# regicide211212/multi-style-transfer-gan

Measured on AMD Instinct MI355X. Metric: train-step images/sec (fwd+bwd+loss), 256x256 batch32, higher is better.
Workload: dtype f32; 1 GPU; config 3: reference CycleGAN train_step (2x EnhancedGenerator + 2x EnhancedDiscriminator, channels=16, num_transformer_blocks=0), 32 image pairs/GPU at 256x256, fwd+bwd+loss+Adam; per_gpu_batch=32, size=256, channels=16, parallelism=dp1, collective=none, losses_finite=True

## Files before the change

multi-style-transfer-gan_amd/mstg_hip/csrc/common.h:

```cpp
#pragma once
#include <hip/hip_runtime.h>
#include <stdint.h>
#include <stdio.h>
#include <string.h>

#include "mstg_hip.h"

typedef float f32x4 __attribute__((ext_vector_type(4)));
typedef float f32x2 __attribute__((ext_vector_type(2)));

namespace mstg {

extern thread_local char g_last_error[256];
inline int fail_launch(hipError_t e, const char* what) {
    snprintf(g_last_error, sizeof(g_last_error), "%s: %s", what, hipGetErrorString(e));
    return MSTG_E_LAUNCH;
}
inline int fail_arg(int code, const char* what) {
    snprintf(g_last_error, sizeof(g_last_error), "%s", what);
    return code;
}
#define MSTG_CHECK_LAUNCH(what)                                   \
    do {                                                          \
        hipError_t e__ = hipGetLastError();                       \
        if (e__ != hipSuccess) return mstg::fail_launch(e__, what); \
    } while (0)

extern bool g_prof_on;
void prof_begin(const void* host_fn, hipStream_t st);
void prof_end(hipStream_t st);
#define MSTG_LAUNCH(kern, grid, block, lds, st, ...)                               \
    do {                                                                           \
        const bool prof__ = mstg::g_prof_on;                                       \
        if (prof__) mstg::prof_begin((const void*)(kern), (hipStream_t)(st));      \
        hipLaunchKernelGGL(kern, grid, block, lds, st, __VA_ARGS__);               \
        if (prof__) mstg::prof_end((hipStream_t)(st));                             \
    } while (0)

extern thread_local bool t_ws_packed;
#define MSTG_PACK_LAUNCH(...)                      \
    do {                                           \
        if (!mstg::t_ws_packed) MSTG_LAUNCH(__VA_ARGS__); \
    } while (0)

enum EnvKnob {
    ENV_ATTN_BLK4, ENV_ATTN_BLK64, ENV_WGRAD_1X1, ENV_WGRAD_TS_MAXCH, ENV_WGRAD_PLAIN, ENV_WGRAD_OLD, ENV_NO_DPACK, ENV_IGEMM,
    ENV_STREAM, ENV_PF, ENV_WGLOB, ENV_HEAVY_PER_CU, ENV_DBG, ENV_DBG_LDS_KB, ENV_MS_WGRAD_PACKED, ENV_MS_FWD4, ENV_NO_PACK_CACHE,
    ENV_P32, ENV_P32_TH, ENV_P32_WLDS, ENV_P32_DBG, ENV_P32_OCC, ENV_ATTN_REG, ENV_NFW_ADAPT, ENV_BSUMS_ALL, ENV_ATTN_BIG32, ENV_NORM_WGS,
    ENV_CONV_IMG, ENV_COUNT
};
const char* env_get(EnvKnob k);

int cu_count();
struct OccCache {
    const void* kern = nullptr;
    size_t lds = 0;
    int occ = 1;
};
int persistent_occupancy(OccCache& c, const void* kern, size_t lds);

constexpr int WAVE = 64;

__device__ __forceinline__ f32x4 mfma16(float a, float b, f32x4 c) {
    return __builtin_amdgcn_mfma_f32_16x16x4f32(a, b, c, 0, 0, 0);
}

__device__ __forceinline__ float wave_sum(float v) {
#pragma unroll
    for (int o = 32; o > 0; o >>= 1) v += __shfl_xor(v, o, 64);
    return v;
}

__device__ __forceinline__ float apply_act(float v, int act) {
    switch (act) {
        case MSTG_ACT_RELU: return v > 0.f ? v : 0.f;
        case MSTG_ACT_LEAKY02: return v > 0.f ? v : 0.2f * v;
        case MSTG_ACT_TANH: return tanhf(v);
        case MSTG_ACT_GELU: return 0.5f * v * (1.f + erff(v * 0.70710678118654752f));
        default: return v;
    }
}
__device__ __forceinline__ float act_grad(float v, int act) {
    switch (act) {
        case MSTG_ACT_RELU: return v > 0.f ? 1.f : 0.f;
        case MSTG_ACT_LEAKY02: return v > 0.f ? 1.f : 0.2f;
        case MSTG_ACT_TANH: return 1.f - v * v;
        case MSTG_ACT_GELU: return 0.5f * (1.f + erff(v * 0.70710678118654752f)) + v * 0.3989422804014327f * expf(-0.5f * v * v);
        default: return 1.f;
    }
}

__device__ __forceinline__ int xcd_swizzle(int bid, int nblk) {
    const int q = nblk >> 3, r = nblk & 7, xcd = bid & 7, k = bid >> 3;
    return (xcd < r ? xcd * (q + 1) : r * (q + 1) + (xcd - r) * q) + k;
}


__host__ __device__ __forceinline__ unsigned magic_u32(unsigned d) { return 0xFFFFFFFFu / d + 1u; }

template <int NB>
__device__ __forceinline__ void stage_window_batch(const float* __restrict__ img, float* __restrict__ lds, int total, int e0, int cols,
                                                   int nq, unsigned m_cols, unsigned m_nq, int y0, int x0, int H, int W, int ctot,
                                                   int nq_valid, int ckp, int tid, int rowpad) {
    f32x4 v[NB];
    int dst[NB];
    bool ok[NB];
#pragma unroll
    for (int k = 0; k < NB; ++k) {
        const int e = e0 + 256 * k + tid;
        const int p = nq == 1 ? e : (int)__umulhi((unsigned)e, m_nq);
        const int q = e - p * nq;
        const int r = (int)__umulhi((unsigned)p, m_cols), c = p - r * cols;
        const int iy = y0 + r, ix = x0 + c;
        ok[k] = e < total && (unsigned)iy < (unsigned)H && (unsigned)ix < (unsigned)W && q < nq_valid;
        const unsigned off = ok[k] ? (unsigned)(iy * W + ix) * (unsigned)ctot + 4u * q : 0u;
        v[k] = *reinterpret_cast<const f32x4*>(img + off);
        dst[k] = e < total ? p * ckp + 4 * q + r * rowpad : -1;
    }
#pragma unroll
    for (int k = 0; k < NB; ++k)
        if (dst[k] >= 0) *reinterpret_cast<f32x4*>(&lds[dst[k]]) = ok[k] ? v[k] : f32x4{0.f, 0.f, 0.f, 0.f};
}

__device__ __forceinline__ void stage_window(const float* __restrict__ img, float* __restrict__ lds, int rows, int cols, int nq,
                                             unsigned m_cols, unsigned m_nq, int y0, int x0, int H, int W, int ctot, int nq_valid,
                                             int ckp, int tid, int rowpad = 0) {
    const int total = rows * cols * nq;
    int e0 = 0;
    for (; e0 + 1024 < total; e0 += 2048)
        stage_window_batch<8>(img, lds, total, e0, cols, nq, m_cols, m_nq, y0, x0, H, W, ctot, nq_valid, ckp, tid, rowpad);
    for (; e0 < total; e0 += 1024)
        stage_window_batch<4>(img, lds, total, e0, cols, nq, m_cols, m_nq, y0, x0, H, W, ctot, nq_valid, ckp, tid, rowpad);
// ... 38 lines not shown
```

multi-style-transfer-gan_amd/mstg_hip/csrc/msblock.hip:

```cpp
#include "common.h"
#include <stdlib.h>

namespace mstg {

constexpr int MS_TH = 8, MS_PH = MS_TH + 8, MS_PW = 16 + 8, MS_CKP = 20;

template <int CH>
__global__ __launch_bounds__(256) void wgrad_ms_kernel(const float* __restrict__ x, const float* __restrict__ dy,
                                                       float* __restrict__ partial, int N, int H, int W, int tiles_x, int tiles_y,
                                                       int ntiles) {
    constexpr int NFH = CH / 16, C4 = CH / 4, U = NFH + 24, UW = (U + 3) / 4, BNP = CH + 4, NG = CH / 16;
    constexpr int PSTRIDE = NG * U * 256 + CH;
    extern __shared__ __attribute__((aligned(16))) float smem[];
    float* patch = smem;
    float* ht = smem + MS_PH * MS_PW * MS_CKP;

    const int tid = threadIdx.x, lane = tid & 63, wave = tid >> 6, i = lane & 15, g = lane >> 4;
    const int gchunk = blockIdx.y, g0 = 16 * gchunk;

    f32x4 acc[UW];
    int toff[UW], hfo[UW];
#pragma unroll
    for (int k = 0; k < UW; ++k) {
        const int u = min(wave + 4 * k, U - 1);
        int dyp = 0, dxp = 0, frag = u;
        if (u >= NFH) {
            const int r = (u - NFH) >> 3, i8 = (u - NFH) & 7, t9 = i8 < 4 ? i8 : i8 + 1, d = 1 << r;
            dyp = (t9 / 3 - 1) * d;
            dxp = (t9 % 3 - 1) * d;
            frag = ((r + 1) * C4) / 16;
        }
        toff[k] = ((4 + dyp) * MS_PW + 4 + dxp) * MS_CKP;
        hfo[k] = 16 * frag;
        acc[k] = f32x4{0.f, 0.f, 0.f, 0.f};
    }
    const int nu = (U - wave + 3) / 4;

    const bool do_bias = gchunk == 0;
    float bsum = 0.f;
    const unsigned m_pw = magic_u32(MS_PW), m_nq = magic_u32(CH / 4);
    const size_t plane = (size_t)H * W;
    for (int tile = blockIdx.x; tile < ntiles; tile += gridDim.x) {
        const int tx0 = tile % tiles_x, ty0 = (tile / tiles_x) % tiles_y, n = tile / (tiles_x * tiles_y);
        __syncthreads();
        stage_window(x + (size_t)n * plane * CH + g0, patch, MS_PH, MS_PW, 4, m_pw, 0x40000000u, ty0 * MS_TH - 4, tx0 * 16 - 4, H, W, CH, 4,
                     MS_CKP, tid);
        stage_window(dy + (size_t)n * plane * CH, ht, MS_TH, 16, CH / 4, 0x10000000u, m_nq, ty0 * MS_TH, tx0 * 16, H, W, CH, CH / 4, BNP, tid);
        __syncthreads();
        if (do_bias && tid < CH) {
#pragma unroll 8
            for (int p = 0; p < MS_TH * 16; ++p) bsum += ht[p * BNP + tid];
        }
#pragma unroll 1
        for (int r = 0; r < MS_TH; ++r) {
#pragma unroll 2
            for (int xs = 0; xs < 4; ++xs) {
                const int c = 4 * xs + g;
                const int abase = (r * MS_PW + c) * MS_CKP + i;
                const int hbase = (r * 16 + c) * BNP + i;
                float af[UW], bf[UW];
#pragma unroll
                for (int k = 0; k < UW; ++k) { af[k] = patch[abase + toff[k]]; bf[k] = ht[hbase + hfo[k]]; }
#pragma unroll
                for (int k = 0; k < UW; ++k) acc[k] = mfma16(af[k], bf[k], acc[k]);
            }
        }
    }
    float* out = partial + (size_t)blockIdx.x * PSTRIDE;
    if (do_bias && tid < CH) out[NG * U * 256 + tid] = bsum;
#pragma unroll
    for (int k = 0; k < UW; ++k) {
        if (k >= nu) continue;
        const int u = wave + 4 * k;
        float* o = out + ((size_t)gchunk * U + u) * 256;
#pragma unroll
        for (int e = 0; e < 4; ++e) o[(4 * g + e) * 16 + i] = acc[k][e];
    }
}

template <int CH>
struct MsUnits {
    static constexpr int NFW = CH / 16, C4 = CH / 4, U = NFW + 24;
    __host__ __device__ static constexpr int ring(int u) { return (u - NFW) >> 3; }
    __host__ __device__ static constexpr int t9(int u) { return ((u - NFW) & 7) < 4 ? ((u - NFW) & 7) : ((u - NFW) & 7) + 1; }
    __host__ __device__ static constexpr int oy(int u) { return u < NFW ? 0 : (t9(u) / 3 - 1) * (1 << ring(u)); }
    __host__ __device__ static constexpr int ox(int u) { return u < NFW ? 0 : (t9(u) % 3 - 1) * (1 << ring(u)); }
    __host__ __device__ static constexpr int frag(int u) { return u < NFW ? u : ((ring(u) + 1) * C4) / 16; }
};

struct MsParamPtrs {
    const float* w[4];
// ... 146 lines not shown
        for (int wf = 0; wf < NFW; ++wf) a[wf] = *reinterpret_cast<const f32x4*>(wpc + ((wf * K::NQ + Q) * 64 + lane) * 4);
#pragma unroll
        for (int e = 0; e < 4; ++e) {
            constexpr int s0 = 4 * Q;
            const int s = s0 + e;
            if (s < K::NS) {
                const int off = (K::oy(s) * MS_PW + K::ox(s)) * MS_CKP + 4 * K::grp(s);
                float b[2];
#pragma unroll
                for (int pf = 0; pf < 2; ++pf) b[pf] = patch[pbase + pf * MS_PW * MS_CKP + off];
#pragma unroll
                for (int wf = 0; wf < NFW; ++wf)
#pragma unroll
                    for (int pf = 0; pf < 2; ++pf) acc[wf][pf] = mfma16(a[wf][e], b[pf], acc[wf][pf]);
            }
        }
        MsDgQuadLoop<CH, C, QB + 1, QE>::run(acc, wpc, patch, pbase, lane);
    }
};
template <int CH, int C, int QE>
struct MsDgQuadLoop<CH, C, QE, QE> {
    template <typename ACC>
    static __device__ __forceinline__ void run(ACC&, const float*, const float*, int, int) {}
};

template <int CH, int C, typename ACC>
__device__ __forceinline__ void ms_dgrad_chunk(ACC& acc, const float* __restrict__ dy_img, const float* __restrict__ wp, float* patch,
                                               int ty0, int tx0, int H, int W, unsigned m_pw, int pbase, int tid, int lane) {
    typedef MsDgChunk<CH, C> K;
    constexpr int NFW = CH / 16;
    if (C) __syncthreads();
    stage_window(dy_img + 16 * C, patch, MS_PH, MS_PW, 4, m_pw, 0x40000000u, ty0 * MS_TH - 4, tx0 * 16 - 4, H, W, CH, 4, MS_CKP, tid);
    __syncthreads();
    MsDgQuadLoop<CH, C, 0, K::NQ>::run(acc, wp + (size_t)ms_dg_quads_before<CH>(C) * NFW * 256, patch, pbase, lane);
}

template <int CH>
__global__ __launch_bounds__(256) void ms_dgrad_kernel(const float* __restrict__ dy, const float* __restrict__ wp,
                                                       const float* __restrict__ dres, float* __restrict__ dx, int N, int H, int W,
                                                       int tiles_x, int tiles_y) {
    constexpr int NFW = CH / 16, PF = 2;
    extern __shared__ __attribute__((aligned(16))) float smem[];
    float* patch = smem;
    const int tid = threadIdx.x, lane = tid & 63, wave = tid >> 6, i = lane & 15, g = lane >> 4;
    const int tile = xcd_swizzle(blockIdx.x, gridDim.x);
    const int tx0 = tile % tiles_x, ty0 = (tile / tiles_x) % tiles_y, n = tile / (tiles_x * tiles_y);
    const size_t plane = (size_t)H * W;
    const unsigned m_pw = magic_u32(MS_PW);
    f32x4 acc[NFW][PF];
#pragma unroll
    for (int wf = 0; wf < NFW; ++wf)
#pragma unroll
        for (int pf = 0; pf < PF; ++pf) acc[wf][pf] = f32x4{0.f, 0.f, 0.f, 0.f};
    const int pbase = ((PF * wave + 4) * MS_PW + i + 4) * MS_CKP + g;
    const float* dy_img = dy + (size_t)n * plane * CH;
    ms_dgrad_chunk<CH, 0>(acc, dy_img, wp, patch, ty0, tx0, H, W, m_pw, pbase, tid, lane);
    if (CH >= 32) ms_dgrad_chunk<CH, (CH >= 32 ? 1 : 0)>(acc, dy_img, wp, patch, ty0, tx0, H, W, m_pw, pbase, tid, lane);
    if (CH >= 64) {
        ms_dgrad_chunk<CH, (CH >= 64 ? 2 : 0)>(acc, dy_img, wp, patch, ty0, tx0, H, W, m_pw, pbase, tid, lane);
        ms_dgrad_chunk<CH, (CH >= 64 ? 3 : 0)>(acc, dy_img, wp, patch, ty0, tx0, H, W, m_pw, pbase, tid, lane);
    }
#pragma unroll
    for (int pf = 0; pf < PF; ++pf) {
        const int gy = ty0 * MS_TH + PF * wave + pf, gx = tx0 * 16 + i;
        if (gy < H && gx < W) {
            const size_t o = (((size_t)n * H + gy) * W + gx) * CH + 4 * g;
#pragma unroll
            for (int wf = 0; wf < NFW; ++wf) {
                f32x4 v = acc[wf][pf];
                if (dres) v += *reinterpret_cast<const f32x4*>(dres + o + 16 * wf);
                *reinterpret_cast<f32x4*>(dx + o + 16 * wf) = v;
            }
        }
    }
}

template <int CH>
struct MsPk {
    static constexpr int NFH = CH / 16, C4 = CH / 4, TPU = 16 / C4, UPB = 8 / TPU, U = NFH + 3 * UPB, UW = (U + 3) / 4;
    static constexpr int NG = CH / 16, PSTRIDE = NG * U * 256 + CH, LDY = CH + 4;
};

template <int CH>
__global__ __launch_bounds__(256) void wgrad_msp_kernel(const float* __restrict__ x, const float* __restrict__ dy,
                                                        float* __restrict__ partial, int N, int H, int W, int tiles_x, int tiles_y,
                                                        int ntiles) {
    typedef MsPk<CH> G;
    constexpr int UW = G::UW, U = G::U, LDY = G::LDY, MG = G::NG, LDX = CH + 4;
    extern __shared__ __attribute__((aligned(16))) float smem[];
    float* xs = smem;
    float* dyp = smem + MS_TH * 16 * LDX;

    const int tid = threadIdx.x, lane = tid & 63, wave = tid >> 6, i = lane & 15, g = lane >> 4;

    f32x4 acc[UW][MG];
    int boff[UW];
#pragma unroll
    for (int k = 0; k < UW; ++k) {
        const int u = min(wave + 4 * k, U - 1);
        int off;
        if (u < G::NFH) {
            off = 16 * u + i;
        } else {
            const int j = 1 + (u - G::NFH) / G::UPB, m = (u - G::NFH) % G::UPB;
            const int sidx = i / G::C4, co = i % G::C4, i8 = m * G::TPU + sidx, t9 = i8 < 4 ? i8 : i8 + 1, d = 1 << (j - 1);
            const int oy = (t9 / 3 - 1) * d, ox = (t9 % 3 - 1) * d;
            off = (-oy * MS_PW - ox) * LDY + j * G::C4 + co;
        }
        boff[k] = off;
#pragma unroll
        for (int mf = 0; mf < MG; ++mf) acc[k][mf] = f32x4{0.f, 0.f, 0.f, 0.f};
    }
    const int nu = (U - wave + 3) / 4;

    float bsum = 0.f;
    const unsigned m_pw = magic_u32(MS_PW), m_nq = magic_u32(CH / 4);
    const size_t plane = (size_t)H * W;
    for (int tile = blockIdx.x; tile < ntiles; tile += gridDim.x) {
        const int tx0 = tile % tiles_x, ty0 = (tile / tiles_x) % tiles_y, n = tile / (tiles_x * tiles_y);
        __syncthreads();
        stage_window(x + (size_t)n * plane * CH, xs, MS_TH, 16, CH / 4, 0x10000000u, m_nq, ty0 * MS_TH, tx0 * 16, H, W, CH, CH / 4, LDX, tid);
        stage_window(dy + (size_t)n * plane * CH, dyp, MS_PH, MS_PW, CH / 4, m_pw, m_nq, ty0 * MS_TH - 4, tx0 * 16 - 4, H, W, CH, CH / 4, LDY,
                     tid);
        __syncthreads();
        if (tid < CH) {
            for (int r = 0; r < MS_TH; ++r)
#pragma unroll 8
                for (int c = 0; c < 16; ++c) bsum += dyp[((r + 4) * MS_PW + c + 4) * LDY + tid];
        }
#pragma unroll 1
        for (int r = 0; r < MS_TH; ++r) {
#pragma unroll 2
            for (int xs4 = 0; xs4 < 4; ++xs4) {
                const int c = 4 * xs4 + g;
                float af[MG], bf[UW];
#pragma unroll
                for (int mf = 0; mf < MG; ++mf) af[mf] = xs[(r * 16 + c) * LDX + 16 * mf + i];
                const int bbase = ((r + 4) * MS_PW + c + 4) * LDY;
#pragma unroll
                for (int k = 0; k < UW; ++k) bf[k] = dyp[bbase + boff[k]];
#pragma unroll
                for (int k = 0; k < UW; ++k)
#pragma unroll
                    for (int mf = 0; mf < MG; ++mf) acc[k][mf] = mfma16(af[mf], bf[k], acc[k][mf]);
            }
        }
    }
    float* out = partial + (size_t)blockIdx.x * G::PSTRIDE;
    if (tid < CH) out[G::NG * U * 256 + tid] = bsum;
#pragma unroll
    for (int k = 0; k < UW; ++k) {
        if (k >= nu) continue;
        const int u = wave + 4 * k;
#pragma unroll
        for (int mf = 0; mf < MG; ++mf) {
            float* o = out + ((size_t)mf * U + u) * 256;
#pragma unroll
            for (int e = 0; e < 4; ++e) o[(4 * g + e) * 16 + i] = acc[k][mf][e];
        }
    }
}

constexpr int M4_TH = 16, M4_PH = M4_TH + 8;

template <int CH, int JB, int T9, int Q>
struct Ms4Step {
    static constexpr int C4 = CH / 4, RS = C4 / 4;
    static __device__ __forceinline__ void run(f32x4 (&acc)[4][RS], const float* __restrict__ wl, const float* __restrict__ patch, int pbase,
                                               int wbase) {
        constexpr int d = JB == 0 ? 0 : (1 << (JB - 1));
        constexpr int oy = JB == 0 ? 0 : (T9 / 3 - 1) * d, ox = JB == 0 ? 0 : (T9 % 3 - 1) * d;
        constexpr int t = JB == 0 ? 0 : 1 + 9 * (JB - 1) + T9;
        const f32x4 b = *reinterpret_cast<const f32x4*>(&patch[pbase + (oy * MS_PW + ox) * MS_CKP + 4 * Q]);
#pragma unroll
        for (int rs = 0; rs < RS; ++rs) {
            const f32x4 a = *reinterpret_cast<const f32x4*>(&wl[wbase + (t * C4 + 4 * rs) * CH + 4 * Q]);
#pragma unroll
            for (int e = 0; e < 4; ++e) acc[JB][rs] = __builtin_amdgcn_mfma_f32_4x4x1f32(a[e], b[e], acc[JB][rs], 0, 0, 0);
        }
    }
};

template <int CH, int JB>
struct Ms4Branch {
    static constexpr int RS = CH / 16;
    static __device__ __forceinline__ void run(f32x4 (&acc)[4][RS], const float* wl, const float* patch, int pbase, int wbase) {
#define M4_TAP(T9)                                                  \
    Ms4Step<CH, JB, T9, 0>::run(acc, wl, patch, pbase, wbase);      \
    Ms4Step<CH, JB, T9, 1>::run(acc, wl, patch, pbase, wbase);      \
    Ms4Step<CH, JB, T9, 2>::run(acc, wl, patch, pbase, wbase);      \
    Ms4Step<CH, JB, T9, 3>::run(acc, wl, patch, pbase, wbase);
        if (JB == 0) {
            M4_TAP(0)
        } else {
            M4_TAP(0) M4_TAP(1) M4_TAP(2) M4_TAP(3) M4_TAP(4) M4_TAP(5) M4_TAP(6) M4_TAP(7) M4_TAP(8)
        }
#undef M4_TAP
    }
};

template <int CH>
__global__ __launch_bounds__(256) void ms_fwd4_kernel(const float* __restrict__ x, MsParamPtrs prm, float* __restrict__ y, int N, int H,
                                                      int W, int tiles_x, int tiles_y) {
    constexpr int C4 = CH / 4, RS = C4 / 4, NCHK = CH / 16;
    extern __shared__ __attribute__((aligned(16))) float smem[];
    float* patch = smem;
    float* wl = smem + M4_PH * MS_PW * MS_CKP;
    const int tid = threadIdx.x, lane = tid & 63, wave = tid >> 6;
    const int tile = xcd_swizzle(blockIdx.x, gridDim.x);
    const int tx0 = tile % tiles_x, ty0 = (tile / tiles_x) % tiles_y, n = tile / (tiles_x * tiles_y);
    const size_t plane = (size_t)H * W;
    for (int e = tid; e < 28 * C4 * CH; e += 256) {
        const int ci = e % CH, co = (e / CH) % C4, t = e / (CH * C4);
        float v;
        if (t == 0) v = prm.w[0][co * CH + ci];
        else v = prm.w[1 + (t - 1) / 9][(co * CH + ci) * 9 + (t - 1) % 9];
        wl[e] = v;
    }
    const int b = lane >> 2, j = lane & 3;
    const int prow = 4 * wave + (b >> 2), pcol = 4 * (b & 3) + j;
    const int pbase = ((prow + 4) * MS_PW + pcol + 4) * MS_CKP;
    f32x4 acc[4][RS];
#pragma unroll
    for (int jb = 0; jb < 4; ++jb)
#pragma unroll
        for (int rs = 0; rs < RS; ++rs) acc[jb][rs] = *reinterpret_cast<const f32x4*>(prm.b[jb] + 4 * rs);
    const unsigned m_pw = magic_u32(MS_PW);
#pragma unroll
    for (int chunk = 0; chunk < NCHK; ++chunk) {
        if (chunk) __syncthreads();
        stage_window(x + (size_t)n * plane * CH + 16 * chunk, patch, M4_PH, MS_PW, 4, m_pw, 0x40000000u, ty0 * M4_TH - 4, tx0 * 16 - 4, H, W,
                     CH, 4, MS_CKP, tid);
        __syncthreads();
        const int wbase = j * CH + 16 * chunk;
        Ms4Branch<CH, 0>::run(acc, wl, patch, pbase, wbase);
        Ms4Branch<CH, 1>::run(acc, wl, patch, pbase, wbase);
        Ms4Branch<CH, 2>::run(acc, wl, patch, pbase, wbase);
        Ms4Branch<CH, 3>::run(acc, wl, patch, pbase, wbase);
    }
    const int gy = ty0 * M4_TH + prow, gx = tx0 * 16 + pcol;
    if (gy < H && gx < W) {
        float* p = y + (((size_t)n * H + gy) * W + gx) * CH;
// ... 218 lines not shown
        const int co = 16 * ((j * C4) / 16) + n;
        if (co >= j * C4 && co < (j + 1) * C4) {
            float* o = &out.dw[j][((co - j * C4) * CH + ci) * 9 + t9];
            *o = accumulate ? *o + r : r;
        }
    }
}

template <int CH>
__global__ __launch_bounds__(256) void wgrad_msp_reduce_kernel(const float* __restrict__ partial, MsGradPtrs out, int S, int accumulate) {
    typedef MsPk<CH> G;
    constexpr int NACC = G::NG * G::U * 256, PSTRIDE = G::PSTRIDE, C4 = G::C4;
    __shared__ float sh[16][17];
    const int e = threadIdx.x & 15, row = threadIdx.x >> 4;
    const int idx = blockIdx.x * 16 + e;
    float sum = 0.f;
    if (idx < PSTRIDE) {
        int sp = row;
        for (; sp + 7 * 16 < S; sp += 8 * 16) {
            float v[8];
#pragma unroll
            for (int k = 0; k < 8; ++k) v[k] = partial[(size_t)(sp + 16 * k) * PSTRIDE + idx];
#pragma unroll
            for (int k = 0; k < 8; ++k) sum += v[k];
        }
        for (; sp < S; sp += 16) sum += partial[(size_t)sp * PSTRIDE + idx];
    }
    sh[row][e] = sum;
    __syncthreads();
    if (row != 0 || idx >= PSTRIDE) return;
    float r = 0.f;
#pragma unroll
    for (int k = 0; k < 16; ++k) r += sh[k][e];
    float* o;
    if (idx >= NACC) {
        const int co = idx - NACC;
        o = &out.db[co / C4][co % C4];
    } else {
        const int n = idx & 15, m = (idx >> 4) & 15, u = (idx >> 8) % G::U, gch = idx / (G::U * 256);
        const int ci = 16 * gch + m;
        if (u < G::NFH) {
            const int co = 16 * u + n, j = co / C4, cj = co % C4;
            o = j == 0 ? &out.dw[0][cj * CH + ci] : &out.dw[j][(cj * CH + ci) * 9 + 4];
        } else {
            const int j = 1 + (u - G::NFH) / G::UPB, mm = (u - G::NFH) % G::UPB;
            const int sidx = n / C4, co = n % C4, i8 = mm * G::TPU + sidx, t9 = i8 < 4 ? i8 : i8 + 1;
            o = &out.dw[j][(co * CH + ci) * 9 + t9];
        }
    }
    *o = accumulate ? *o + r : r;
}

template <int CH>
static bool ms_wgrad_packed() {
    const char* e = env_get(ENV_MS_WGRAD_PACKED);
    return CH <= 32 && !(e && e[0] == '0');
}

template <int CH>
static size_t ms_wgrad_plan(int N, int H, int W, int& S, int& tiles_x, int& tiles_y, int& ntiles) {
    constexpr int NFH = CH / 16, U = NFH + 24, NG = CH / 16, PSTRIDE = NG * U * 256 + CH;
    tiles_x = cdiv(W, 16);
    tiles_y = cdiv(H, MS_TH);
    ntiles = N * tiles_x * tiles_y;
    S = 768 / NG;
    if (S > ntiles) S = ntiles;
    if (S < 1) S = 1;
    size_t need = (size_t)S * PSTRIDE;
    if (CH <= 32) {
        const size_t sp = (size_t)S * NG > (size_t)ntiles ? (size_t)ntiles : (size_t)S * NG;
        const size_t np = sp * MsPk<(CH <= 32 ? CH : 16)>::PSTRIDE;
        if (np > need) need = np;
    }
    return need * sizeof(float);
}

template <int CH>
static int launch_ms_wgrad(const float* x, const float* dy, const MsGradPtrs& out, int accumulate, int N, int H, int W, void* ws,
                           size_t ws_bytes, hipStream_t st) {
    constexpr int NFH = CH / 16, U = NFH + 24, NG = CH / 16, PSTRIDE = NG * U * 256 + CH;
    int S, tiles_x, tiles_y, ntiles;
    const size_t need = ms_wgrad_plan<CH>(N, H, W, S, tiles_x, tiles_y, ntiles);
    if (!ws || ws_bytes < need) return fail_arg(MSTG_E_WORKSPACE, "msblock_wgrad: workspace too small");
    const size_t lds = (size_t)(MS_PH * MS_PW * MS_CKP + MS_TH * 16 * (CH + 4)) * sizeof(float);
    static bool attr_set = false;
    if (!attr_set) {
        hipError_t e = hipFuncSetAttribute(reinterpret_cast<const void*>(&wgrad_ms_kernel<CH>), hipFuncAttributeMaxDynamicSharedMemorySize,
                                           160 * 1024);
        if (e != hipSuccess) return fail_launch(e, "hipFuncSetAttribute(wgrad_ms)");
        attr_set = true;
    }
    if (ms_wgrad_packed<CH>()) {
        typedef MsPk<CH> P;
        const size_t ldsp = (size_t)(MS_TH * 16 * (CH + 4) + MS_PH * MS_PW * P::LDY) * sizeof(float);
        static bool attr_set_p = false;
        if (!attr_set_p) {
            hipError_t e = hipFuncSetAttribute(reinterpret_cast<const void*>(&wgrad_msp_kernel<CH>),
                                               hipFuncAttributeMaxDynamicSharedMemorySize, 160 * 1024);
            if (e != hipSuccess) return fail_launch(e, "hipFuncSetAttribute(wgrad_msp)");
            attr_set_p = true;
        }
        const int Sp = S * NG > ntiles ? ntiles : S * NG;
        MSTG_LAUNCH((wgrad_msp_kernel<CH>), dim3(Sp, 1, 1), dim3(256), ldsp, st, x, dy, (float*)ws, N, H, W, tiles_x, tiles_y, ntiles);
        MSTG_CHECK_LAUNCH("wgrad_msp_kernel");
        MSTG_LAUNCH((wgrad_msp_reduce_kernel<CH>), dim3(cdiv(P::PSTRIDE, 16)), dim3(256), 0, st, (const float*)ws, out, Sp, accumulate);
        MSTG_CHECK_LAUNCH("wgrad_msp_reduce_kernel");
        return MSTG_OK;
    }
    MSTG_LAUNCH((wgrad_ms_kernel<CH>), dim3(S, NG, 1), dim3(256), lds, st, x, dy, (float*)ws, N, H, W, tiles_x, tiles_y, ntiles);
    MSTG_CHECK_LAUNCH("wgrad_ms_kernel");
    MSTG_LAUNCH((wgrad_ms_reduce_kernel<CH>), dim3(cdiv(PSTRIDE, 16)), dim3(256), 0, st, (const float*)ws, out, S, accumulate);
    MSTG_CHECK_LAUNCH("wgrad_ms_reduce_kernel");
    return MSTG_OK;
}

template <int CH>
static int launch_ms_fwd(const float* x, const MsParamPtrs& prm, float* y, int N, int H, int W, void* ws, size_t ws_bytes, hipStream_t st) {
    typedef MsUnits<CH> G;
    {
        const char* e = env_get(ENV_MS_FWD4);
        bool aligned = true;
        for (int k = 0; k < 4; ++k) aligned = aligned && (reinterpret_cast<uintptr_t>(prm.b[k]) & 15) == 0;
        const bool use4b = CH <= 32 && (!e || e[0] == '3');
        const bool use4 = !use4b && ((CH == 16 && !(e && e[0] == '0')) || (CH == 32 && e && e[0] == '2'));
        if ((use4 || use4b) && aligned && H >= 16) {
            constexpr int C4K = (CH <= 32 ? CH : 16);
            const int tiles_x = cdiv(W, 16), tiles_y = cdiv(H, M4_TH);
            constexpr int LDW4B = C4K == 16 ? C4K : C4K + 4;
            const size_t lds = use4b ? (size_t)(M4_PH * M4B_ROW + 28 * (C4K / 4) * LDW4B) * sizeof(float)
                                     : (size_t)(M4_PH * MS_PW * MS_CKP + 28 * (C4K / 4) * C4K) * sizeof(float);
            static bool attr4 = false;
            if (!attr4) {
                hipError_t er = hipFuncSetAttribute(reinterpret_cast<const void*>(&ms_fwd4_kernel<C4K>),
                                                    hipFuncAttributeMaxDynamicSharedMemorySize, 160 * 1024);
                if (er == hipSuccess)
                    er = hipFuncSetAttribute(reinterpret_cast<const void*>(&ms_fwd4b_kernel<C4K>), hipFuncAttributeMaxDynamicSharedMemorySize,
                                             160 * 1024);
                if (er != hipSuccess) return fail_launch(er, "hipFuncSetAttribute(ms_fwd4)");
                attr4 = true;
            }
            if (use4b) {
                constexpr int PACKED = 28 * (C4K / 4) * LDW4B + C4K;
                if (!ws || ws_bytes < (size_t)PACKED * sizeof(float)) return fail_arg(MSTG_E_WORKSPACE, "msblock_fwd: workspace too small");
                MSTG_PACK_LAUNCH((ms_pack_fwd4b_kernel<C4K>), dim3(cdiv(PACKED, 256)), dim3(256), 0, st, prm, (float*)ws);
                MSTG_CHECK_LAUNCH("ms_pack_fwd4b_kernel");
                const int ntiles = N * tiles_x * tiles_y, slots = (C4K == 16 ? 3 : 2) * cu_count();
                MSTG_LAUNCH((ms_fwd4b_kernel<C4K>), dim3(ntiles < slots ? ntiles : slots), dim3(256), lds, st, x, (const float*)ws, y, N, H, W,
                            tiles_x, tiles_y, ntiles);
            } else MSTG_LAUNCH((ms_fwd4_kernel<C4K>), dim3(N * tiles_x * tiles_y), dim3(256), lds, st, x, prm, y, N, H, W, tiles_x, tiles_y);
            MSTG_CHECK_LAUNCH("ms_fwd4_kernel");
            return MSTG_OK;
        }
    }
    constexpr int NCH = CH / 16;
    const size_t need = (size_t)(NCH * G::U * 256 + CH) * sizeof(float);
    if (!ws || ws_bytes < need) return fail_arg(MSTG_E_WORKSPACE, "msblock_fwd: workspace too small");
    float* wp = (float*)ws;
    MSTG_PACK_LAUNCH((ms_pack_fwd_kernel<CH>), dim3(cdiv(NCH * G::U * 256 + CH, 256)), dim3(256), 0, st, prm, wp);
    MSTG_CHECK_LAUNCH("ms_pack_fwd_kernel");
    const int tiles_x = cdiv(W, 16), tiles_y = cdiv(H, MS_TH);
    const size_t lds = (size_t)(MS_PH * MS_PW * MS_CKP) * sizeof(float);
    MSTG_LAUNCH((ms_fwd_kernel<CH>), dim3(N * tiles_x * tiles_y), dim3(256), lds, st, x, (const float*)wp, y, N, H, W, tiles_x,
                       tiles_y);
    MSTG_CHECK_LAUNCH("ms_fwd_kernel");
    return MSTG_OK;
}

template <int CH>
static size_t ms_dgrad_ws_floats() {
    return (size_t)ms_dg_quads_before<CH>(CH / 16) * (CH / 16) * 256;
}

template <int CH>
static int launch_ms_dgrad(const float* dy, const MsParamPtrs& prm, const float* dres, float* dx, int N, int H, int W, void* ws,
                           size_t ws_bytes, hipStream_t st) {
    const size_t need = ms_dgrad_ws_floats<CH>() * sizeof(float);
    if (!ws || ws_bytes < need) return fail_arg(MSTG_E_WORKSPACE, "msblock_dgrad: workspace too small");
    float* wp = (float*)ws;
    MSTG_PACK_LAUNCH((ms_pack_dgrad_kernel<CH>), dim3(cdiv((int)ms_dgrad_ws_floats<CH>(), 1024)), dim3(256), 0, st, prm, wp);
    MSTG_CHECK_LAUNCH("ms_pack_dgrad_kernel");
    const int tiles_x = cdiv(W, 16), tiles_y = cdiv(H, MS_TH);
    const size_t lds = (size_t)(MS_PH * MS_PW * MS_CKP) * sizeof(float);
    MSTG_LAUNCH((ms_dgrad_kernel<CH>), dim3(N * tiles_x * tiles_y), dim3(256), lds, st, dy, (const float*)wp, dres, dx, N, H, W,
                       tiles_x, tiles_y);
    MSTG_CHECK_LAUNCH("ms_dgrad_kernel");
    return MSTG_OK;
}

}

using namespace mstg;

// ... 81 lines not shown
```

multi-style-transfer-gan_amd/mstg_hip/csrc/runtime.hip:

```cpp
#include <stdlib.h>

#include <cxxabi.h>

#include <mutex>
#include <string>
#include <vector>

#include "common.h"

namespace mstg {

thread_local char g_last_error[256] = "";
thread_local bool t_ws_packed = false;

static const char* const kEnvNames[ENV_COUNT] = {
    "MSTG_ATTN_BLK4", "MSTG_ATTN_BLK64", "MSTG_WGRAD_1X1", "MSTG_WGRAD_TS_MAXCH", "MSTG_WGRAD_PLAIN", "MSTG_WGRAD_OLD", "MSTG_NO_DPACK",
    "MSTG_IGEMM", "MSTG_STREAM", "MSTG_PF", "MSTG_WGLOB", "MSTG_HEAVY_PER_CU", "MSTG_DBG", "MSTG_DBG_LDS_KB", "MSTG_MS_WGRAD_PACKED",
    "MSTG_MS_FWD4", "MSTG_NO_PACK_CACHE", "MSTG_P32", "MSTG_P32_TH", "MSTG_P32_WLDS", "MSTG_P32_DBG", "MSTG_P32_OCC", "MSTG_ATTN_REG", "MSTG_NFW_ADAPT", "MSTG_BSUMS_ALL", "MSTG_ATTN_BIG32", "MSTG_NORM_WGS",
    "MSTG_CONV_IMG"};

struct EnvCache {
    char val[ENV_COUNT][32];
    bool set[ENV_COUNT];
    EnvCache() { refresh(); }
    void refresh() {
        for (int k = 0; k < ENV_COUNT; ++k) {
            const char* e = getenv(kEnvNames[k]);
            set[k] = e != nullptr;
            snprintf(val[k], sizeof(val[k]), "%s", e ? e : "");
        }
    }
};
static EnvCache g_env;

const char* env_get(EnvKnob k) { return g_env.set[k] ? g_env.val[k] : nullptr; }

int cu_count() {
    static int cus = 0;
    if (!cus) {
        int dev = 0;
        hipDeviceProp_t p;
        if (hipGetDevice(&dev) == hipSuccess && hipGetDeviceProperties(&p, dev) == hipSuccess) cus = p.multiProcessorCount;
        if (cus <= 0) cus = 256;
    }
    return cus;
}

int persistent_occupancy(OccCache& c, const void* kern, size_t lds) {
    if (c.kern != kern || c.lds != lds) {
        if (lds > 64 * 1024) (void)hipFuncSetAttribute(kern, hipFuncAttributeMaxDynamicSharedMemorySize, 160 * 1024);
        int nb = 1;
        if (hipOccupancyMaxActiveBlocksPerMultiprocessor(&nb, kern, 256, lds) != hipSuccess || nb < 1) nb = 1;
        c.occ = nb > 4 ? 4 : nb;
        c.kern = kern;
        c.lds = lds;
    }
    return c.occ;
}

bool g_prof_on = false;
struct ProfRec {
    const void* fn;
    hipStream_t st;
    hipEvent_t e0, e1;
};
static std::vector<ProfRec> g_prof;
static std::mutex g_prof_mu;
static thread_local int t_prof_open = -1;

void prof_begin(const void* fn, hipStream_t st) {
    ProfRec r{fn, st, nullptr, nullptr};
    if (hipEventCreate(&r.e0) != hipSuccess || hipEventCreate(&r.e1) != hipSuccess) return;
    (void)hipEventRecord(r.e0, st);
    std::lock_guard<std::mutex> lk(g_prof_mu);
    t_prof_open = (int)g_prof.size();
    g_prof.push_back(r);
}
void prof_end(hipStream_t st) {
    std::lock_guard<std::mutex> lk(g_prof_mu);
    if (t_prof_open < 0 || t_prof_open >= (int)g_prof.size()) return;
    (void)hipEventRecord(g_prof[t_prof_open].e1, st);
    t_prof_open = -1;
}
static void prof_clear() {
    for (auto& r : g_prof) {
        (void)hipEventDestroy(r.e0);
        (void)hipEventDestroy(r.e1);
    }
    g_prof.clear();
}

}

extern "C" const char* mstg_version(void) { return "mstg-hip 0.2.0 gfx950"; }
extern "C" const char* mstg_arch(void) { return "gfx950"; }
extern "C" const char* mstg_last_error(void) { return mstg::g_last_error; }
extern "C" void mstg_env_refresh(void) { mstg::g_env.refresh(); }

extern "C" int mstg_prof_enable(int on) {
    std::lock_guard<std::mutex> lk(mstg::g_prof_mu);
    if (on) mstg::prof_clear();
    mstg::g_prof_on = on != 0;
// ... 34 lines not shown
```

Baseline: 1723 images/sec.

## Prefetch next tile into registers in multi-scale wgrad kernels

Adds register-prefetched versions of the multi-scale weight-gradient kernels. Each workgroup loads the next tile's x and dy windows into registers while it runs MFMA products on the current tile from LDS, and uses a fast unguarded path for interior tiles. The change also moves to tighter LDS pitches, adds occupancy launch bounds and rotates wave roles across blocks. The old synchronous kernels stay available behind an environment switch, and the prefetch path is the default. The cost is more register pressure, which could lower occupancy.

```diff
diff --git a/multi-style-transfer-gan_amd/mstg_hip/csrc/common.h b/multi-style-transfer-gan_amd/mstg_hip/csrc/common.h
--- a/multi-style-transfer-gan_amd/mstg_hip/csrc/common.h
+++ b/multi-style-transfer-gan_amd/mstg_hip/csrc/common.h
@@ -47,7 +47,7 @@
     ENV_ATTN_BLK4, ENV_ATTN_BLK64, ENV_WGRAD_1X1, ENV_WGRAD_TS_MAXCH, ENV_WGRAD_PLAIN, ENV_WGRAD_OLD, ENV_NO_DPACK, ENV_IGEMM,
     ENV_STREAM, ENV_PF, ENV_WGLOB, ENV_HEAVY_PER_CU, ENV_DBG, ENV_DBG_LDS_KB, ENV_MS_WGRAD_PACKED, ENV_MS_FWD4, ENV_NO_PACK_CACHE,
     ENV_P32, ENV_P32_TH, ENV_P32_WLDS, ENV_P32_DBG, ENV_P32_OCC, ENV_ATTN_REG, ENV_NFW_ADAPT, ENV_BSUMS_ALL, ENV_ATTN_BIG32, ENV_NORM_WGS,
-    ENV_CONV_IMG, ENV_COUNT
+    ENV_CONV_IMG, ENV_MS_WGRAD_PF, ENV_COUNT
 };
 const char* env_get(EnvKnob k);
 
diff --git a/multi-style-transfer-gan_amd/mstg_hip/csrc/msblock.hip b/multi-style-transfer-gan_amd/mstg_hip/csrc/msblock.hip
--- a/multi-style-transfer-gan_amd/mstg_hip/csrc/msblock.hip
+++ b/multi-style-transfer-gan_amd/mstg_hip/csrc/msblock.hip
@@ -6,7 +6,7 @@
 constexpr int MS_TH = 8, MS_PH = MS_TH + 8, MS_PW = 16 + 8, MS_CKP = 20;
 
 template <int CH>
-__global__ __launch_bounds__(256) void wgrad_ms_kernel(const float* __restrict__ x, const float* __restrict__ dy,
+__global__ __launch_bounds__(256) void wgrad_ms_sync_kernel(const float* __restrict__ x, const float* __restrict__ dy,
                                                        float* __restrict__ partial, int N, int H, int W, int tiles_x, int tiles_y,
                                                        int ntiles) {
     constexpr int NFH = CH / 16, C4 = CH / 4, U = NFH + 24, UW = (U + 3) / 4, BNP = CH + 4, NG = CH / 16;
@@ -319,7 +319,7 @@
 };
 
 template <int CH>
-__global__ __launch_bounds__(256) void wgrad_msp_kernel(const float* __restrict__ x, const float* __restrict__ dy,
+__global__ __launch_bounds__(256) void wgrad_msp_sync_kernel(const float* __restrict__ x, const float* __restrict__ dy,
                                                         float* __restrict__ partial, int N, int H, int W, int tiles_x, int tiles_y,
                                                         int ntiles) {
     typedef MsPk<CH> G;
@@ -395,6 +395,274 @@
 #pragma unroll
             for (int e = 0; e < 4; ++e) o[(4 * g + e) * 16 + i] = acc[k][mf][e];
         }
+    }
+}
+
+
+template <int ROWS, int COLS, int NQ, int LD>
+struct MsTileWindow {
+    static constexpr int NV = ROWS * COLS * NQ / 256;
+    static_assert(ROWS * COLS * NQ == NV * 256 && NV <= 32, "the window's quads divide evenly over the workgroup");
+    f32x4 v[NV];
+    unsigned rel[NV];
+    unsigned ok;
+    bool full;
+    __device__ __forceinline__ void init(int W, int ctot, int tid) {
+#pragma unroll
+        for (int k = 0; k < NV; ++k) {
+            const unsigned e = 256u * k + tid, p = e / NQ, q = e % NQ, r = p / COLS, c = p % COLS;
+            rel[k] = ((r * W + c) * ctot + 4 * q) * 4u;
+        }
+        ok = 0;
+        full = false;
+    }
+    __device__ __forceinline__ void fetch(const float* __restrict__ img, int y0, int x0, int H, int W, int ctot, int tid) {
+        const int base = (y0 * W + x0) * ctot;
+        full = y0 >= 0 && x0 >= 0 && y0 + ROWS <= H && x0 + COLS <= W;
+        if (full) {
+            const char* t = reinterpret_cast<const char*>(img + base);
+#pragma unroll
+            for (int k = 0; k < NV; ++k) v[k] = *reinterpret_cast<const f32x4*>(t + rel[k]);
+        } else {
+            ok = 0;
+#pragma unroll
+            for (int k = 0; k < NV; ++k) {
+                const unsigned e = 256u * k + tid, p = e / NQ, r = p / COLS, c = p % COLS;
+                const int iy = y0 + (int)r, ix = x0 + (int)c;
+                const bool in = (unsigned)iy < (unsigned)H && (unsigned)ix < (unsigned)W;
+                const unsigned off = in ? (unsigned)(4 * base) + rel[k] : 0u;
+                v[k] = *reinterpret_cast<const f32x4*>(reinterpret_cast<const char*>(img) + off);
+                ok |= (in ? 1u : 0u) << k;
+            }
+        }
+    }
+    __device__ __forceinline__ void commit(float* __restrict__ lds, int tid) const {
+        if (full) {
+#pragma unroll
+            for (int k = 0; k < NV; ++k) {
+                const unsigned e = 256u * k + tid, p = e / NQ, q = e % NQ;
+                *reinterpret_cast<f32x4*>(&lds[p * LD + 4 * q]) = v[k];
+            }
+        } else {
+#pragma unroll
+            for (int k = 0; k < NV; ++k) {
+                const unsigned e = 256u * k + tid, p = e / NQ, q = e % NQ;
+                *reinterpret_cast<f32x4*>(&lds[p * LD + 4 * q]) = ((ok >> k) & 1) ? v[k] : f32x4{0.f, 0.f, 0.f, 0.f};
+            }
+        }
+    }
+};
+
+__device__ __forceinline__ int ms_wave_role(int wave) {
+    const int j = blockIdx.x >> 3;
+    return __builtin_amdgcn_readfirstlane((wave + j + (j >> 5)) & 3);
+}
+
+__host__ __device__ constexpr int ms_op_pitch(int ch) { return ch == 16 ? 16 : ch + 16; }
+
+template <int CH, bool BIAS, int NU>
+__device__ __forceinline__ void msp_tile_products(f32x4 (&acc)[MsPk<CH>::UW][MsPk<CH>::NG], float& bsum, const float* __restrict__ xa,
+                                                  const float* __restrict__ dyl, const int (&bo)[MsPk<CH>::UW], const float* __restrict__ bb) {
+    constexpr int MG = MsPk<CH>::NG, LDY = MsPk<CH>::LDY, LDX = ms_op_pitch(CH);
+#pragma unroll 1
+    for (int r = 0; r < MS_TH; ++r) {
+        float bv[16];
+        if (BIAS) {
+#pragma unroll
+            for (int c = 0; c < 16; ++c) bv[c] = bb[(r * MS_PW + c) * LDY];
+        }
+#pragma unroll
+        for (int xs4 = 0; xs4 < 4; ++xs4) {
+            float af[MG], bf[NU];
+#pragma unroll
+            for (int mf = 0; mf < MG; ++mf) af[mf] = xa[(r * 16 + 4 * xs4) * LDX + 16 * mf];
+#pragma unroll
+            for (int k = 0; k < NU; ++k) bf[k] = dyl[bo[k] + (r * MS_PW + 4 * xs4) * LDY];
+#pragma unroll
+            for (int k = 0; k < NU; ++k)
+#pragma unroll
+                for (int mf = 0; mf < MG; ++mf) acc[k][mf] = mfma16(af[mf], bf[k], acc[k][mf]);
+        }
+        if (BIAS) {
+#pragma unroll
+            for (int c = 0; c < 16; ++c) bsum += bv[c];
+        }
+    }
+}
+
+template <int CH>
+__global__ __launch_bounds__(256, CH == 16 ? 4 : 2) void wgrad_msp_kernel(const float* __restrict__ x, const float* __restrict__ dy,
+                                                                          float* __restrict__ partial, int N, int H, int W, int tiles_x,
+                                                                          int tiles_y, int ntiles) {
+    typedef MsPk<CH> G;
+    constexpr int UW = G::UW, U = G::U, LDY = G::LDY, MG = G::NG, LDX = ms_op_pitch(CH);
+    constexpr int NUS = U % 4 ? UW - 1 : UW;
+    extern __shared__ __attribute__((aligned(16))) float smem[];
+    float* xs = smem;
+    float* dyp = smem + MS_TH * 16 * LDX;
+
+    const int tid = threadIdx.x, lane = tid & 63, i = lane & 15, g = lane >> 4;
+    const int role = ms_wave_role(tid >> 6);
+
+    f32x4 acc[UW][MG];
+    int bo[UW];
+#pragma unroll
+    for (int k = 0; k < UW; ++k) {
+        const int u = min(role + 4 * k, U - 1);
+        int off;
+        if (u < G::NFH) {
+            off = 16 * u;
+        } else {
+            const int j = 1 + (u - G::NFH) / G::UPB, m = (u - G::NFH) % G::UPB;
+            const int sidx = i / G::C4, co = i % G::C4, i8 = m * G::TPU + sidx, t9 = i8 < 4 ? i8 : i8 + 1, d = 1 << (j - 1);
+            const int oy = (t9 / 3 - 1) * d, ox = (t9 % 3 - 1) * d;
+            off = (-oy * MS_PW - ox) * LDY + j * G::C4 + co - i;
+        }
+        bo[k] = off;
+#pragma unroll
+        for (int mf = 0; mf < MG; ++mf) acc[k][mf] = f32x4{0.f, 0.f, 0.f, 0.f};
+    }
+    const bool short_wave = U % 4 != 0 && role >= U % 4, bias_wave = role >= 4 - CH / 16;
+    static_assert(U % 4 == 0 || 4 - CH / 16 >= U % 4, "the bias waves are short waves");
+    const int bch = 16 * (role - (4 - CH / 16)) + i;
+    const float* xa = xs + g * LDX + i;
+    const float* dyl = dyp + (4 * MS_PW + 4 + g) * LDY + i;
+    const float* bb = dyp + (4 * MS_PW + 4) * LDY + (bias_wave ? bch : 0);
+
+    float bsum = 0.f;
+    const size_t plane = (size_t)H * W;
+    MsTileWindow<MS_TH, 16, CH / 4, LDX> wx;
+    MsTileWindow<MS_PH, MS_PW, CH / 4, LDY> wd;
+    wx.init(W, CH, tid);
+    wd.init(W, CH, tid);
+    auto fetch = [&](int tile) {
+        const int tx0 = tile % tiles_x, ty0 = (tile / tiles_x) % tiles_y, n = tile / (tiles_x * tiles_y);
+        wx.fetch(x + (size_t)n * plane * CH, ty0 * MS_TH, tx0 * 16, H, W, CH, tid);
+        wd.fetch(dy + (size_t)n * plane * CH, ty0 * MS_TH - 4, tx0 * 16 - 4, H, W, CH, tid);
+    };
+    if ((int)blockIdx.x < ntiles) fetch(blockIdx.x);
+    for (int tile = blockIdx.x; tile < ntiles; tile += gridDim.x) {
+        __syncthreads();
+        wx.commit(xs, tid);
+        wd.commit(dyp, tid);
+        __syncthreads();
+        if (tile + (int)gridDim.x < ntiles) fetch(tile + gridDim.x);
+        if (bias_wave) msp_tile_products<CH, true, NUS>(acc, bsum, xa, dyl, bo, bb);
+        else if (NUS != UW && short_wave) msp_tile_products<CH, false, NUS>(acc, bsum, xa, dyl, bo, bb);
+        else msp_tile_products<CH, false, UW>(acc, bsum, xa, dyl, bo, bb);
+    }
+    float* out = partial + (size_t)blockIdx.x * G::PSTRIDE;
+    if (bias_wave && g == 0) out[G::NG * U * 256 + bch] = bsum;
+    const int nu = (U - role + 3) / 4;
+#pragma unroll
+    for (int k = 0; k < UW; ++k) {
+        if (k >= nu) continue;
+        const int u = role + 4 * k;
+#pragma unroll
+        for (int mf = 0; mf < MG; ++mf) {
+            float* o = out + ((size_t)mf * U + u) * 256;
+#pragma unroll
+            for (int e = 0; e < 4; ++e) o[(4 * g + e) * 16 + i] = acc[k][mf][e];
+        }
+    }
+}
+
+template <int CH, bool BIAS, int NU, int UW>
+__device__ __forceinline__ void ms_tile_products(f32x4 (&acc)[UW], float& bsum, const float* __restrict__ patch, const float* __restrict__ ht,
+                                                 const int (&ao)[UW], const int (&ho)[UW], const float* __restrict__ bb) {
+    constexpr int BNP = ms_op_pitch(CH), CKP = 16;
+#pragma unroll 1
+    for (int r = 0; r < MS_TH; ++r) {
+        float bv[16];
+        if (BIAS) {
+#pragma unroll
+            for (int c = 0; c < 16; ++c) bv[c] = bb[(r * 16 + c) * BNP];
+        }
+#pragma unroll
+        for (int xs4 = 0; xs4 < 4; ++xs4) {
+            float af[NU], bf[NU];
+#pragma unroll
+            for (int k = 0; k < NU; ++k) {
+                af[k] = patch[ao[k] + (r * MS_PW + 4 * xs4) * CKP];
+                bf[k] = ht[ho[k] + (r * 16 + 4 * xs4) * BNP];
+            }
+#pragma unroll
+            for (int k = 0; k < NU; ++k) acc[k] = mfma16(af[k], bf[k], acc[k]);
+        }
+        if (BIAS) {
+#pragma unroll
+            for (int c = 0; c < 16; ++c) bsum += bv[c];
+        }
+    }
+}
+
+template <int CH>
+__global__ __launch_bounds__(256, 2) void wgrad_ms_kernel(const float* __restrict__ x, const float* __restrict__ dy,
+                                                          float* __restrict__ partial, int N, int H, int W, int tiles_x, int tiles_y,
+                                                          int ntiles) {
+    constexpr int NFH = CH / 16, C4 = CH / 4, U = NFH + 24, UW = (U + 3) / 4, BNP = ms_op_pitch(CH), CKP = 16, NG = CH / 16;
+    constexpr int PSTRIDE = NG * U * 256 + CH, NUS = U % 4 ? UW - 1 : UW;
+    extern __shared__ __attribute__((aligned(16))) float smem[];
+    float* patch = smem;
+    float* ht = smem + MS_PH * MS_PW * CKP;
+
+    const int tid = threadIdx.x, lane = tid & 63, i = lane & 15, g = lane >> 4;
+    const int role = ms_wave_role(tid >> 6);
+    const int gchunk = blockIdx.y, g0 = 16 * gchunk;
+
+    f32x4 acc[UW];
+    int ao[UW], ho[UW];
+#pragma unroll
+    for (int k = 0; k < UW; ++k) {
+        const int u = min(role + 4 * k, U - 1);
+        int dyp = 0, dxp = 0, frag = u;
+        if (u >= NFH) {
+            const int r = (u - NFH) >> 3, i8 = (u - NFH) & 7, t9 = i8 < 4 ? i8 : i8 + 1, d = 1 << r;
+            dyp = (t9 / 3 - 1) * d;
+            dxp = (t9 % 3 - 1) * d;
+            frag = ((r + 1) * C4) / 16;
+        }
+        ao[k] = ((4 + dyp) * MS_PW + 4 + dxp + g) * CKP + i;
+        ho[k] = g * BNP + 16 * frag + i;
+        acc[k] = f32x4{0.f, 0.f, 0.f, 0.f};
+    }
+    const bool short_wave = U % 4 != 0 && role >= U % 4, bias_wave = gchunk == 0 && role >= 4 - CH / 16;
+    static_assert(U % 4 == 0 || 4 - CH / 16 >= U % 4, "the bias waves are short waves");
+    const int bch = 16 * (role - (4 - CH / 16)) + i;
+    const float* bb = ht + (bias_wave ? bch : 0);
+
+    float bsum = 0.f;
+    const size_t plane = (size_t)H * W;
+    MsTileWindow<MS_PH, MS_PW, 4, CKP> wx;
+    MsTileWindow<MS_TH, 16, CH / 4, BNP> wd;
+    wx.init(W, CH, tid);
+    wd.init(W, CH, tid);
+    auto fetch = [&](int tile) {
+        const int tx0 = tile % tiles_x, ty0 = (tile / tiles_x) % tiles_y, n = tile / (tiles_x * tiles_y);
+        wx.fetch(x + (size_t)n * plane * CH + g0, ty0 * MS_TH - 4, tx0 * 16 - 4, H, W, CH, tid);
+        wd.fetch(dy + (size_t)n * plane * CH, ty0 * MS_TH, tx0 * 16, H, W, CH, tid);
+    };
+    if ((int)blockIdx.x < ntiles) fetch(blockIdx.x);
+    for (int tile = blockIdx.x; tile < ntiles; tile += gridDim.x) {
+        __syncthreads();
+        wx.commit(patch, tid);
+        wd.commit(ht, tid);
+        __syncthreads();
+        if (tile + (int)gridDim.x < ntiles) fetch(tile + gridDim.x);
+        if (bias_wave) ms_tile_products<CH, true, NUS, UW>(acc, bsum, patch, ht, ao, ho, bb);
+        else if (NUS != UW && short_wave) ms_tile_products<CH, false, NUS, UW>(acc, bsum, patch, ht, ao, ho, bb);
+        else ms_tile_products<CH, false, UW, UW>(acc, bsum, patch, ht, ao, ho, bb);
+    }
+    float* out = partial + (size_t)blockIdx.x * PSTRIDE;
+    if (bias_wave && g == 0) out[NG * U * 256 + bch] = bsum;
+    const int nu = (U - role + 3) / 4;
+#pragma unroll
+    for (int k = 0; k < UW; ++k) {
+        if (k >= nu) continue;
+        const int u = role + 4 * k;
+        float* o = out + ((size_t)gchunk * U + u) * 256;
+#pragma unroll
+        for (int e = 0; e < 4; ++e) o[(4 * g + e) * 16 + i] = acc[k][e];
     }
 }
 
@@ -779,32 +1047,37 @@
     int S, tiles_x, tiles_y, ntiles;
     const size_t need = ms_wgrad_plan<CH>(N, H, W, S, tiles_x, tiles_y, ntiles);
     if (!ws || ws_bytes < need) return fail_arg(MSTG_E_WORKSPACE, "msblock_wgrad: workspace too small");
-    const size_t lds = (size_t)(MS_PH * MS_PW * MS_CKP + MS_TH * 16 * (CH + 4)) * sizeof(float);
-    static bool attr_set = false;
-    if (!attr_set) {
-        hipError_t e = hipFuncSetAttribute(reinterpret_cast<const void*>(&wgrad_ms_kernel<CH>), hipFuncAttributeMaxDynamicSharedMemorySize,
-                                           160 * 1024);
-        if (e != hipSuccess) return fail_launch(e, "hipFuncSetAttribute(wgrad_ms)");
-        attr_set = true;
-    }
+    typedef void (*kern_t)(const float*, const float*, float*, int, int, int, int, int, int);
+    const char* epf = env_get(ENV_MS_WGRAD_PF);
+    const int pf = !(epf && epf[0] == '0');
+    const size_t lds =
+        (size_t)(pf ? MS_PH * MS_PW * 16 + MS_TH * 16 * ms_op_pitch(CH) : MS_PH * MS_PW * MS_CKP + MS_TH * 16 * (CH + 4)) * sizeof(float);
     if (ms_wgrad_packed<CH>()) {
-        typedef MsPk<CH> P;
-        const size_t ldsp = (size_t)(MS_TH * 16 * (CH + 4) + MS_PH * MS_PW * P::LDY) * sizeof(float);
-        static bool attr_set_p = false;
-        if (!attr_set_p) {
-            hipError_t e = hipFuncSetAttribute(reinterpret_cast<const void*>(&wgrad_msp_kernel<CH>),
-                                               hipFuncAttributeMaxDynamicSharedMemorySize, 160 * 1024);
+        typedef MsPk<(CH <= 32 ? CH : 16)> P;
+        constexpr int CP = CH <= 32 ? CH : 16;
+        const size_t ldsp = (size_t)(MS_TH * 16 * (pf ? ms_op_pitch(CH) : CH + 4) + MS_PH * MS_PW * P::LDY) * sizeof(float);
+        const kern_t kern = pf ? &wgrad_msp_kernel<CP> : &wgrad_msp_sync_kernel<CP>;
+        static bool attr_set_p[2] = {false, false};
+        if (!attr_set_p[pf]) {
+            hipError_t e = hipFuncSetAttribute(reinterpret_cast<const void*>(kern), hipFuncAttributeMaxDynamicSharedMemorySize, 160 * 1024);
             if (e != hipSuccess) return fail_launch(e, "hipFuncSetAttribute(wgrad_msp)");
-            attr_set_p = true;
+            attr_set_p[pf] = true;
         }
         const int Sp = S * NG > ntiles ? ntiles : S * NG;
-        MSTG_LAUNCH((wgrad_msp_kernel<CH>), dim3(Sp, 1, 1), dim3(256), ldsp, st, x, dy, (float*)ws, N, H, W, tiles_x, tiles_y, ntiles);
+        MSTG_LAUNCH(kern, dim3(Sp, 1, 1), dim3(256), ldsp, st, x, dy, (float*)ws, N, H, W, tiles_x, tiles_y, ntiles);
         MSTG_CHECK_LAUNCH("wgrad_msp_kernel");
-        MSTG_LAUNCH((wgrad_msp_reduce_kernel<CH>), dim3(cdiv(P::PSTRIDE, 16)), dim3(256), 0, st, (const float*)ws, out, Sp, accumulate);
+        MSTG_LAUNCH((wgrad_msp_reduce_kernel<CP>), dim3(cdiv(P::PSTRIDE, 16)), dim3(256), 0, st, (const float*)ws, out, Sp, accumulate);
         MSTG_CHECK_LAUNCH("wgrad_msp_reduce_kernel");
         return MSTG_OK;
     }
-    MSTG_LAUNCH((wgrad_ms_kernel<CH>), dim3(S, NG, 1), dim3(256), lds, st, x, dy, (float*)ws, N, H, W, tiles_x, tiles_y, ntiles);
+    const kern_t kern = pf ? &wgrad_ms_kernel<CH> : &wgrad_ms_sync_kernel<CH>;
+    static bool attr_set[2] = {false, false};
+    if (!attr_set[pf]) {
+        hipError_t e = hipFuncSetAttribute(reinterpret_cast<const void*>(kern), hipFuncAttributeMaxDynamicSharedMemorySize, 160 * 1024);
+        if (e != hipSuccess) return fail_launch(e, "hipFuncSetAttribute(wgrad_ms)");
+        attr_set[pf] = true;
+    }
+    MSTG_LAUNCH(kern, dim3(S, NG, 1), dim3(256), lds, st, x, dy, (float*)ws, N, H, W, tiles_x, tiles_y, ntiles);
     MSTG_CHECK_LAUNCH("wgrad_ms_kernel");
     MSTG_LAUNCH((wgrad_ms_reduce_kernel<CH>), dim3(cdiv(PSTRIDE, 16)), dim3(256), 0, st, (const float*)ws, out, S, accumulate);
     MSTG_CHECK_LAUNCH("wgrad_ms_reduce_kernel");
diff --git a/multi-style-transfer-gan_amd/mstg_hip/csrc/runtime.hip b/multi-style-transfer-gan_amd/mstg_hip/csrc/runtime.hip
--- a/multi-style-transfer-gan_amd/mstg_hip/csrc/runtime.hip
+++ b/multi-style-transfer-gan_amd/mstg_hip/csrc/runtime.hip
@@ -17,7 +17,7 @@
     "MSTG_ATTN_BLK4", "MSTG_ATTN_BLK64", "MSTG_WGRAD_1X1", "MSTG_WGRAD_TS_MAXCH", "MSTG_WGRAD_PLAIN", "MSTG_WGRAD_OLD", "MSTG_NO_DPACK",
     "MSTG_IGEMM", "MSTG_STREAM", "MSTG_PF", "MSTG_WGLOB", "MSTG_HEAVY_PER_CU", "MSTG_DBG", "MSTG_DBG_LDS_KB", "MSTG_MS_WGRAD_PACKED",
     "MSTG_MS_FWD4", "MSTG_NO_PACK_CACHE", "MSTG_P32", "MSTG_P32_TH", "MSTG_P32_WLDS", "MSTG_P32_DBG", "MSTG_P32_OCC", "MSTG_ATTN_REG", "MSTG_NFW_ADAPT", "MSTG_BSUMS_ALL", "MSTG_ATTN_BIG32", "MSTG_NORM_WGS",
-    "MSTG_CONV_IMG"};
+    "MSTG_CONV_IMG", "MSTG_MS_WGRAD_PF"};
 
 struct EnvCache {
     char val[ENV_COUNT][32];
```

Result: faster. 1743 images/sec, median of 6 (+1.2%).
